# flynn-nrg/izpi

Hardware: AMD Instinct MI355X
Metric: Msamples/sec (pixels x spp) at 1024x1024/512spp (higher is better)
Workload: dtype f64

## Files before the change

### include/izpi_gpu_debug.h

```cpp
#ifndef IZPI_GPU_DEBUG_H
#define IZPI_GPU_DEBUG_H
#include "izpi_gpu.h"

#ifdef __cplusplus
extern "C" {
#endif

int izpi_gpu_debug_fault(izpi_ctx* ctx, int where);

int izpi_gpu_debug_realloc(izpi_ctx* ctx, uint32_t mask);

#ifdef __cplusplus
}
#endif
#endif
```

### izpi_amd/_native.py

```python
import ctypes as C
from pathlib import Path

ROOT = Path(__file__).resolve().parents[1]
LIB_PATH = ROOT / "izpi_amd" / "_lib" / "libizpi_gpu.so"

c_double_p = C.POINTER(C.c_double)
c_uint32_p = C.POINTER(C.c_uint32)
c_float_p = C.POINTER(C.c_float)

COMM_ID_BYTES = 128
IZPI_OK, IZPI_ERR_INVALID, IZPI_ERR_HIP, IZPI_ERR_NO_SCENE, IZPI_ERR_UNSUPPORTED, IZPI_ERR_DEVICE, IZPI_ERR_PEER = range(7)
IZPI_ABI_VERSION = 4
ACC_RECURSIVE, ACC_FORWARD = 0, 1
SCENE_QUANTIZED_BVH = 1
PRIM_TRIANGLE, PRIM_SPHERE = 0, 1
TEX_CONSTANT, TEX_IMAGE, TEX_SPECTRAL_GAUSSIAN, TEX_SPECTRAL_TABULATED, TEX_SPECTRAL_IMAGE = 1, 3, 5, 7, 9
MAT_DIELECTRIC, MAT_DIFFUSE_LIGHT, MAT_ISOTROPIC, MAT_LAMBERT, MAT_METAL, MAT_PBR = 1, 2, 3, 4, 5, 6
MATF_BEER_LAMBERT = 1
SAMPLER_NORMAL, SAMPLER_COLOUR, SAMPLER_WIREFRAME, SAMPLER_ALBEDO, SAMPLER_SPECTRAL = 1, 2, 3, 4, 5
OUT_CANVAS, OUT_PACKED = 0, 1
POST_NONE, POST_SPECTRAL, POST_GAMMA_CLAMP = 0, 1, 2
SNAP_CANVAS, SNAP_DISPLAY, SNAP_NOISE = 0, 1, 2
PROG_NOISE = 1
PROG_ADAPTIVE = 4
# ... 206 lines not shown
    _fields_ = [("name", C.c_char_p), ("kd", C.c_double * 3), ("ka", C.c_double * 3), ("ks", C.c_double * 3),
                ("num_kd", C.c_uint32), ("num_ka", C.c_uint32), ("num_ks", C.c_uint32), ("pad", C.c_uint32),
                ("ns", C.c_double), ("ni", C.c_double), ("d", C.c_double), ("sharpness", C.c_int64),
                ("illum", C.c_int64)]


ABI_STRUCTS = [BVH4Node, Texture, Material, Camera, SceneDesc, RenderReq, RenderStats, Hit, TriIn, SphereIn, CameraIn,
               SceneInput, ProtoInfo, ObjInfo, ObjGroup, ObjMaterial, RenderTuning, DenoiseParams, NoiseParams, NoiseStats, AdaptStats]

EXPORTS = [
    "izpi_gpu_open", "izpi_gpu_close", "izpi_gpu_prepare", "izpi_gpu_multi_prepare", "izpi_gpu_last_error", "izpi_gpu_upload_scene", "izpi_gpu_render",
    "izpi_gpu_render_device", "izpi_gpu_unpack_tiles", "izpi_gpu_output_bytes", "izpi_gpu_trace",
    "izpi_gpu_ray_aabb4", "izpi_gpu_gomath", "izpi_gpu_spectral_post", "izpi_gpu_postprocess",
    "izpi_gpu_build_bvh4", "izpi_gpu_multi_open", "izpi_gpu_multi_close", "izpi_gpu_multi_last_error",
    "izpi_gpu_multi_size", "izpi_gpu_multi_context", "izpi_gpu_multi_upload_scene", "izpi_gpu_multi_render",
    "izpi_gpu_comm_id", "izpi_gpu_comm_init", "izpi_gpu_render_rank", "izpi_gpu_debug_fault", "izpi_gpu_debug_realloc", "izpi_gpu_progress", "izpi_gpu_multi_progress", "izpi_host_build_scene_ex", "izpi_host_scene_prim_boxes", "izpi_host_scene_set_bvh", "izpi_host_scene_set_flags",
    "izpi_host_build_scene", "izpi_host_scene_desc", "izpi_host_scene_stack_bound", "izpi_host_scene_build_ms",
    "izpi_host_scene_free", "izpi_host_last_error", "izpi_host_tiles", "izpi_host_share_units", "izpi_host_share_tiles", "izpi_host_share_block", "izpi_host_assemble_shares", "izpi_host_bvh_leaf_max", "izpi_host_gomath", "izpi_abi_struct_size",
    "izpi_scene_parse_text", "izpi_scene_parse_binary", "izpi_scene_serialize", "izpi_scene_info", "izpi_scene_image_file",
    "izpi_scene_set_image", "izpi_scene_add_triangles", "izpi_scene_background", "izpi_scene_to_input",
    "izpi_scene_material_name", "izpi_scene_free", "izpi_light_source", "izpi_light_source_name",
    "izpi_obj_parse", "izpi_obj_info_get", "izpi_obj_copy_vertices", "izpi_obj_group_get", "izpi_obj_copy_faces",
    "izpi_obj_material_get", "izpi_obj_translate", "izpi_obj_scale", "izpi_obj_rotate",
    "izpi_obj_group_to_triangles", "izpi_obj_free",
    "izpi_gpu_displace", "izpi_host_displace", "izpi_scene_displacement_file", "izpi_scene_set_displacement_map",
    "izpi_scene_set_displacer",
    "izpi_gpu_progressive_begin", "izpi_gpu_progressive_step", "izpi_gpu_progressive_snapshot",
    "izpi_gpu_progressive_snapshot_device", "izpi_gpu_progressive_end",
    "izpi_gpu_multi_progressive_begin", "izpi_gpu_multi_progressive_step", "izpi_gpu_multi_progressive_snapshot",
    "izpi_gpu_multi_progressive_end",
    "izpi_gpu_denoise_device", "izpi_gpu_denoise", "izpi_host_denoise",
# ... 40 lines not shown
    L.izpi_gpu_multi_open.argtypes = [C.POINTER(C.c_int), C.c_uint32, C.POINTER(C.c_void_p)]
    L.izpi_gpu_multi_close.argtypes = [C.c_void_p]
    L.izpi_gpu_multi_last_error.argtypes = [C.c_void_p]
    L.izpi_gpu_multi_last_error.restype = C.c_char_p
    L.izpi_gpu_multi_size.argtypes = [C.c_void_p]
    L.izpi_gpu_multi_size.restype = C.c_uint32
    L.izpi_gpu_multi_context.argtypes = [C.c_void_p, C.c_uint32]
    L.izpi_gpu_multi_context.restype = C.c_void_p
    L.izpi_gpu_multi_upload_scene.argtypes = [C.c_void_p, C.POINTER(SceneDesc)]
    L.izpi_gpu_multi_render.argtypes = [C.c_void_p, C.POINTER(RenderReq), C.c_void_p, C.POINTER(RenderStats)]
    L.izpi_gpu_comm_id.argtypes = [C.POINTER(C.c_uint8)]
    L.izpi_gpu_comm_init.argtypes = [C.c_void_p, C.c_uint32, C.c_uint32, C.POINTER(C.c_uint8)]
    L.izpi_gpu_render_rank.argtypes = [C.c_void_p, C.POINTER(RenderReq), C.c_void_p, C.POINTER(RenderStats)]
    L.izpi_gpu_debug_fault.argtypes = [C.c_void_p, C.c_int]
    L.izpi_gpu_debug_realloc.argtypes = [C.c_void_p, C.c_uint32]
    L.izpi_gpu_progress.argtypes = [C.c_void_p, C.POINTER(C.c_uint64), C.POINTER(C.c_uint64)]
    L.izpi_gpu_multi_progress.argtypes = [C.c_void_p, C.POINTER(C.c_uint64), C.POINTER(C.c_uint64)]
    for pre in ("izpi_gpu_progressive_", "izpi_gpu_multi_progressive_"):
        getattr(L, pre + "begin").argtypes = [C.c_void_p, C.POINTER(RenderReq), C.c_uint32]
        getattr(L, pre + "step").argtypes = [C.c_void_p, C.c_uint32, C.POINTER(RenderStats)]
        getattr(L, pre + "snapshot").argtypes = [C.c_void_p, C.c_uint32, C.c_void_p]
        getattr(L, pre + "end").argtypes = [C.c_void_p]
        getattr(L, pre + "begin_ex").argtypes = [C.c_void_p, C.POINTER(RenderReq), C.c_uint32, C.c_uint32]
        getattr(L, pre + "noise").argtypes = [C.c_void_p, C.POINTER(NoiseParams), C.POINTER(NoiseStats)]
        getattr(L, pre + "adapt").argtypes = [C.c_void_p, C.POINTER(NoiseParams), C.POINTER(AdaptStats)]
        getattr(L, pre + "converge").argtypes = [C.c_void_p, C.POINTER(NoiseParams), C.POINTER(RenderStats),
                                                 C.POINTER(NoiseStats)]
    L.izpi_gpu_progressive_snapshot_device.argtypes = [C.c_void_p, C.c_uint32, C.c_void_p]
    L.izpi_host_build_scene_ex.argtypes = [C.POINTER(SceneInput), C.c_uint32, C.POINTER(C.c_void_p)]
    L.izpi_host_scene_prim_boxes.argtypes = [C.c_void_p, c_double_p]
# ... 79 lines not shown
```

### izpi_amd/csrc/components.hip

```cpp
#include "izpi_runtime.h"

using namespace izpi_internal;

__global__ void __launch_bounds__(256) k_spectral_post(const double* in, double* out, uint32_t W, uint32_t H,
                                                       double exposure) {
  __shared__ double ys[18][18];
  const int tx = threadIdx.x & 15, ty = threadIdx.x >> 4;
  const int x0 = blockIdx.x * 16, y0 = blockIdx.y * 16;
  for (int i = threadIdx.x; i < 18 * 18; i += 256) {
    const int hx = x0 + (i % 18) - 1, hy = y0 + (i / 18) - 1;
    ys[i / 18][i % 18] = (hx >= 0 && hx < (int)W && hy >= 0 && hy < (int)H) ? in[((size_t)hy * W + hx) * 4 + 1] : 0.0;
  }
  __syncthreads();
  const int x = x0 + tx, y = y0 + ty;
  if (x >= (int)W || y >= (int)H) return;
  const size_t pi = ((size_t)y * W + x) * 4;
  const double2 xy = *reinterpret_cast<const double2*>(in + pi), za = *reinterpret_cast<const double2*>(in + pi + 2);
  double X = xy.x, Y = xy.y, Z = za.x;
  const double cur = ys[ty + 1][tx + 1];
  if (cur > 0) {
    double nb[8];
    int nn = 0;
    for (int dy = -1; dy <= 1; dy++)
      for (int dx = -1; dx <= 1; dx++) {
// ... 85 lines not shown
  }
  out[i] = h;
}

__global__ void k_aabb4(const float* boxes, const float* rays, uint32_t n, uint8_t* masks) {
  const uint32_t i = blockIdx.x * 256 + threadIdx.x;
  if (i >= n) return;
  const float* b = boxes + (size_t)i * 24;
  const float* r = rays + (size_t)i * 7;
  uint8_t m = 0;
  for (int k = 0; k < 4; k++)
    if (slab(b[k], b[4 + k], b[8 + k], b[12 + k], b[16 + k], b[20 + k], r[0], r[1], r[2], r[3], r[4], r[5], r[6])) m |= (uint8_t)(1 << k);
  masks[i] = m;
}

__global__ void k_gomath(const DevScene sc, int op, const double* x, const double* y, uint32_t n, double* out) {
  const uint32_t i = blockIdx.x * 256 + threadIdx.x;
  if (i >= n) return;
  if (op == 14) {
    out[i] = path_length(mk(x[3 * i], x[3 * i + 1], x[3 * i + 2]), mk(y[3 * i], y[3 * i + 1], y[3 * i + 2]));
    return;
  }
  double a = x[i], b = y ? y[i] : 0.0, r;
  switch (op) {
    case 0: r = gm::sin(a); break;
    case 1: r = gm::cos(a); break;
    case 2: r = gm::tan(a); break;
    case 3: r = gm::exp(a); break;
    case 4: r = gm::log(a); break;
    case 5: r = gm::pow(a, b); break;
// ... 165 lines not shown
  HIP_TRY(hipSetDevice(ctx->device));
  DevBufs tmp;
  float *db, *dr; uint8_t* dm;
  HIP_TRY(tmp.alloc(&db, (size_t)n * 24));
  HIP_TRY(tmp.alloc(&dr, (size_t)n * 7));
  HIP_TRY(tmp.alloc(&dm, n));
  HIP_TRY(hipMemcpy(db, boxes, (size_t)n * 24 * sizeof(float), hipMemcpyHostToDevice));
  HIP_TRY(hipMemcpy(dr, rays, (size_t)n * 7 * sizeof(float), hipMemcpyHostToDevice));
  hipLaunchKernelGGL(k_aabb4, dim3((n + 255) / 256), dim3(256), 0, ctx->stream, db, dr, n, dm);
  HIP_TRY(hipGetLastError());
  HIP_TRY(hipStreamSynchronize(ctx->stream));
  HIP_TRY(hipMemcpy(masks, dm, n, hipMemcpyDeviceToHost));
  return IZPI_OK;
}

int izpi_gpu_gomath(izpi_ctx* ctx, int op, const double* x, const double* y, uint32_t n, double* out) {
  if (!ctx || !x || !out) return IZPI_ERR_INVALID;
  if (n == 0) return IZPI_OK;
  if (op == 37) {
    if (!ctx->have_scene) { ctx->err = "texture lookup before izpi_gpu_upload_scene"; return IZPI_ERR_NO_SCENE; }
    if (!y) { ctx->err = "texture lookup without texture numbers"; return IZPI_ERR_INVALID; }
    for (uint32_t i = 0; i < n; i++)
      if (!(y[i] >= 0 && y[i] < (double)ctx->num_textures)) { ctx->err = "texture number out of range"; return IZPI_ERR_INVALID; }
  }
  if (op == 14 && !y) { ctx->err = "path length without exit points"; return IZPI_ERR_INVALID; }
  const size_t nin = op == 14 ? 3 * (size_t)n : n;
  HIP_TRY(hipSetDevice(ctx->device));
  DevBufs tmp;
  double *dx, *dy = nullptr, *dout;
  HIP_TRY(tmp.alloc(&dx, nin));
// ... 15 lines not shown
```

### izpi_amd/csrc/izpi_dev.h

```cpp
#pragma once
#include <hip/hip_runtime.h>
#include <stdint.h>
#include "../../include/izpi_gpu.h"
#include "gomath.h"
#include "scene_records.h"

#define IZPI_DEV __device__ __forceinline__

namespace izd {

struct DevScene {
  const GInner* inner;
  const GInnerQ* innerq;
  const GLeaf* leaves;
  const GPrim* prims;
  const GShade* shade;
  const GTriTex* tritex;
  const GLight* lights;
  const izpi_material* materials;
  const izpi_texture* textures;
  const double4* mat_const;
  const MatTex* mat_tex;
  const double* texels;
  const double* spd_wl;
  const double* spd_val;
  int32_t root;
  uint32_t num_lights;
  uint32_t nan_free_bounds;
  uint32_t leaf_shortcut;
  uint32_t tri_only;
  uint32_t no_pathlen;
  uint32_t num_inner;
  uint32_t num_prims;
  izpi_camera cam;
  uint32_t lds_bytes;
  uint32_t time_free;
  uint32_t quantized;
  uint32_t addr32;
  uint32_t leaf_max;
#ifdef IZPI_SHADOW
  const GInner* sh_inner;
  const GLeaf* sh_leaves;
  const GPrim* sh_prims;
#endif
};

struct RenderParams {
  uint32_t width, height, spp, max_depth;
  uint32_t chunk_spp;
  uint32_t s0;
  uint32_t num_pixels;
  uint32_t tile_w, tile_h;
  uint32_t total_units;
  uint32_t lanes;
// ... 99 lines not shown
  double phi = 6.283185307179586 * r1;
  double sp, cp;
  gm::sincos_nonneg(phi, &sp, &cp);
  double x = cp * gm::sqrt(1 - z * z);
  double y = sp * gm::sqrt(1 - z * z);
  return mk(x, y, z);
}
IZPI_DEV V3 random_in_unit_sphere(Lcg& r) {
  for (;;) {
    double x = r.next(), y = r.next(), z = r.next();
    V3 p = sub(smul(mk(x, y, z), 2.0), mk(1.0, 1.0, 1.0));
    if (sqlen(p) < 1.0) return p;
  }
}

IZPI_DEV float max32(float a, float b) { return a > b ? a : b; }
IZPI_DEV float min32(float a, float b) { return a < b ? a : b; }
IZPI_DEV bool slab(float mnx, float mny, float mnz, float mxx, float mxy, float mxz, float ox, float oy, float oz,
                   float ix, float iy, float iz, float tmax) {
  float t0x = (mnx - ox) * ix, t1x = (mxx - ox) * ix;
  if (t0x > t1x) { float t = t0x; t0x = t1x; t1x = t; }
  float t0y = (mny - oy) * iy, t1y = (mxy - oy) * iy;
  if (t0y > t1y) { float t = t0y; t0y = t1y; t1y = t; }
  float t0z = (mnz - oz) * iz, t1z = (mxz - oz) * iz;
  if (t0z > t1z) { float t = t0z; t0z = t1z; t1z = t; }
  float tn = max32(max32(t0x, t0y), t0z);
  float tf = min32(min32(t1x, t1y), t1z);
  return tn <= tf && tf >= 0 && tn <= tmax;
}

typedef float f32x2 __attribute__((ext_vector_type(2)));
IZPI_DEV void slab4_fast(float4 mnx, float4 mny, float4 mnz, float4 mxx, float4 mxy, float4 mxz, float ox, float oy,
                         float oz, float ix, float iy, float iz, float tmax, uint64_t (&h)[4]) {
  const f32x2 o_x = {ox, ox}, o_y = {oy, oy}, o_z = {oz, oz};
  const f32x2 i_x = {ix, ix}, i_y = {iy, iy}, i_z = {iz, iz};
  const f32x2 a0x = (f32x2{mnx.x, mnx.y} - o_x) * i_x, a1x = (f32x2{mnx.z, mnx.w} - o_x) * i_x;
  const f32x2 b0x = (f32x2{mxx.x, mxx.y} - o_x) * i_x, b1x = (f32x2{mxx.z, mxx.w} - o_x) * i_x;
  const f32x2 a0y = (f32x2{mny.x, mny.y} - o_y) * i_y, a1y = (f32x2{mny.z, mny.w} - o_y) * i_y;
  const f32x2 b0y = (f32x2{mxy.x, mxy.y} - o_y) * i_y, b1y = (f32x2{mxy.z, mxy.w} - o_y) * i_y;
  const f32x2 a0z = (f32x2{mnz.x, mnz.y} - o_z) * i_z, a1z = (f32x2{mnz.z, mnz.w} - o_z) * i_z;
  const f32x2 b0z = (f32x2{mxz.x, mxz.y} - o_z) * i_z, b1z = (f32x2{mxz.z, mxz.w} - o_z) * i_z;
  const float t0x[4] = {a0x.x, a0x.y, a1x.x, a1x.y}, t1x[4] = {b0x.x, b0x.y, b1x.x, b1x.y};
  const float t0y[4] = {a0y.x, a0y.y, a1y.x, a1y.y}, t1y[4] = {b0y.x, b0y.y, b1y.x, b1y.y};
  const float t0z[4] = {a0z.x, a0z.y, a1z.x, a1z.y}, t1z[4] = {b0z.x, b0z.y, b1z.x, b1z.y};
#pragma unroll
  for (int i = 0; i < 4; i++) {
    const float tn = __builtin_fmaxf(__builtin_fmaxf(__builtin_fminf(t0x[i], t1x[i]), __builtin_fminf(t0y[i], t1y[i])),
                                     __builtin_fminf(t0z[i], t1z[i]));
    const float tf = __builtin_fminf(__builtin_fminf(__builtin_fmaxf(t0x[i], t1x[i]), __builtin_fmaxf(t0y[i], t1y[i])),
                                     __builtin_fmaxf(t0z[i], t1z[i]));
    h[i] = __builtin_amdgcn_ballot_w64(tn <= tf) & __builtin_amdgcn_ballot_w64(tf >= 0.0f) & __builtin_amdgcn_ballot_w64(tn <= tmax);
  }
}
IZPI_DEV bool ray_fast_ok(float ox, float oy, float oz, float ix, float iy, float iz) {
  const float inf = __builtin_huge_valf();
  return __builtin_fabsf(ox) < inf && __builtin_fabsf(oy) < inf && __builtin_fabsf(oz) < inf &&
         __builtin_fabsf(ix) < inf && __builtin_fabsf(iy) < inf && __builtin_fabsf(iz) < inf &&
         ix != 0.0f && iy != 0.0f && iz != 0.0f;
}

IZPI_DEV bool tri_intersect(const double* a, V3 o, V3 d, double tmin, double tmax, double& t, double& u, double& v) {
  const double eps = 1e-8;
  V3 v0 = mk(a[0], a[1], a[2]), e1 = mk(a[3], a[4], a[5]), e2 = mk(a[6], a[7], a[8]);
  V3 h = cross(d, e2);
  double aa = dot(e1, h);
  if (gm::abs(aa) < eps) return false;
  double f = 1.0 / aa;
  V3 s = sub(o, v0);
  u = f * dot(s, h);
  if (u < -eps || u > 1.0 + eps) return false;
  V3 q = cross(s, e1);
  v = f * dot(d, q);
  if (v < -eps || u + v > 1.0 + eps) return false;
// ... 53 lines not shown
```

### izpi_amd/csrc/izpi_gpu.hip

```cpp
#include "izpi_runtime.h"
#include "scene_pack.h"

#include <array>

using namespace izpi_internal;

__global__ void __launch_bounds__(256) k_cpart_reduce(const unsigned long long* cpart, uint32_t rows,
                                                      unsigned long long* counters) {
  __shared__ unsigned long long red[256];
  unsigned long long v = 0;
  for (uint32_t r = threadIdx.x; r < rows; r += 256) v += cpart[(size_t)r * CNT_N + blockIdx.x];
  red[threadIdx.x] = v;
  __syncthreads();
  for (uint32_t h = 128; h > 0; h >>= 1) {
    if (threadIdx.x < h) red[threadIdx.x] += red[threadIdx.x + h];
    __syncthreads();
  }
  if (threadIdx.x == 0) counters[blockIdx.x] += red[0];
}

namespace izpi_internal {
int grow(izpi_ctx* ctx, void** p, size_t* cap, size_t bytes) {
  if (*cap >= bytes) return IZPI_OK;
  if (*p) HIP_TRY(hipFree(*p));
// ... 488 lines not shown
  HIP_TRY(hipSetDevice(ctx->device));
  HIP_TRY(hipStreamSynchronize(ctx->stream));
  free_scene(ctx);
  return IZPI_OK;
}

int upload_packed(izpi_ctx* ctx, const izpi_scene_desc* d, const PackedScene& ps) {
  DevScene& sc = ctx->sc;
  memset(&sc, 0, sizeof(sc));
  GInner* di; GInnerQ* dq; GLeaf* dl; GPrim* dp; GShade* dsh; GTriVerts* dtv; GTriTex* dtt; GLight* dlt;
  izpi_material* dm; Double4* dmc; MatTex* dmt; izpi_texture* dtx;
  double *dtex, *dswl, *dsv;
  {
    const TraceLayout tl = trace_layout(ps.inner.size(), ps.innerq.size(), ps.leaves.size());
    char* nb;
    UP((const char*)nullptr, tl.bytes, &nb);
    di = reinterpret_cast<GInner*>(nb);
    dq = ps.innerq.empty() ? nullptr : reinterpret_cast<GInnerQ*>(nb + tl.innerq_at);
    dl = reinterpret_cast<GLeaf*>(nb + tl.leaves_at);
    HIP_TRY(hipMemcpy(di, ps.inner.data(), ps.inner.size() * sizeof(GInner), hipMemcpyHostToDevice));
    if (dq) HIP_TRY(hipMemcpy(dq, ps.innerq.data(), ps.innerq.size() * sizeof(GInnerQ), hipMemcpyHostToDevice));
    HIP_TRY(hipMemcpy(dl, ps.leaves.data(), ps.leaves.size() * sizeof(GLeaf), hipMemcpyHostToDevice));
  }
  UP(ps.prims.data(), ps.prims.size(), &dp);
  UP(ps.shade.data(), ps.shade.size(), &dsh);
  UP(ps.triverts.data(), ps.triverts.size(), &dtv);
  UP(ps.tritex.data(), ps.tritex.size(), &dtt);
  UP(ps.lights.data(), ps.lights.size(), &dlt);
  UP(d->materials, d->num_materials, &dm);
  UP(ps.mat_const.data(), ps.mat_const.size(), &dmc);
  UP(ps.mat_tex.data(), ps.mat_tex.size(), &dmt);
// ... 3 lines not shown
  UP(d->spd_values, d->num_spd, &dsv);
#ifdef IZPI_SHADOW
  {
    GInner* si; GLeaf* sl; GPrim* sp;
    UP(ps.inner.data(), ps.inner.size(), &si);
    UP(ps.leaves.data(), ps.leaves.size(), &sl);
    UP(ps.prims.data(), ps.prims.size(), &sp);
    sc.sh_inner = si; sc.sh_leaves = sl; sc.sh_prims = sp;
  }
#endif
  sc.inner = di; sc.innerq = dq; sc.leaves = dl; sc.prims = dp; sc.shade = dsh; sc.tritex = dtt; sc.lights = dlt;
  sc.materials = dm; sc.mat_const = (const double4*)dmc; sc.mat_tex = dmt; sc.textures = dtx; sc.texels = dtex;
  sc.spd_wl = dswl; sc.spd_val = dsv;
  sc.root = ps.root; sc.num_inner = ps.num_inner; sc.num_prims = d->num_prims; sc.num_lights = d->num_lights;
  sc.quantized = ps.quantized; sc.leaf_shortcut = ps.leaf_shortcut; sc.nan_free_bounds = ps.nan_free_bounds;
  sc.tri_only = ps.tri_only; sc.time_free = ps.time_free; sc.no_pathlen = ps.no_pathlen; sc.leaf_max = ps.leaf_max;
  sc.addr32 = trace_addr32(ps.inner.size(), ps.innerq.size(), ps.leaves.size(), ps.prims.size());
  sc.cam = d->camera;
  ctx->d_triverts = dtv;
  ctx->mat_ok_rgb = ps.mat_ok_rgb; ctx->mat_ok_spectral = ps.mat_ok_spectral;
  ctx->basic_materials = ps.basic_materials; ctx->matset = ps.matset;
  ctx->const_albedo = ps.const_albedo; ctx->any_uv = ps.any_uv;
  ctx->pool_grow = 0;
  ctx->stack_needed = ps.stack_needed;
  ctx->num_prims = d->num_prims;
  ctx->num_textures = d->num_textures;
  ctx->num_materials = d->num_materials;
  ctx->num_spd = d->num_spd;
  ctx->have_scene = true;
  ctx->plans[0].valid = ctx->plans[1].valid = false;
// ... 150 lines not shown
```

### izpi_amd/csrc/scene_pack.cpp

```cpp
#include "scene_pack.h"

#include <string.h>
#include <algorithm>
#include <cmath>

namespace izpi_internal {

using namespace izd;

bool stack_bound(const izpi_bvh4_node* nodes, size_t n, uint32_t* bound) {
  std::vector<uint32_t> best(n, 0);
  for (size_t k = n; k-- > 0;) {
    const izpi_bvh4_node& nd = nodes[k];
    if (nd.prim_count[0] > 0) continue;
    uint32_t valid = 0, deepest = 0;
    for (int i = 0; i < 4; i++) {
      if (nd.child[i] < 0) continue;
      valid++;
      if ((uint32_t)nd.child[i] <= k) return false;
      deepest = std::max(deepest, best[(size_t)nd.child[i]]);
    }
    best[k] = (valid ? valid - 1 : 0) + deepest;
  }
  *bound = n ? best[0] : 0;
// ... 351 lines not shown
    const double* c0 = d->sph_center0 + 3 * (size_t)i;
    const double* c1 = d->sph_center1 + 3 * (size_t)i;
    const double t0 = d->sph_time[2 * (size_t)i], t1 = d->sph_time[2 * (size_t)i + 1];
    for (int k = 0; k < 3; k++)
      if (!std::isfinite(c0[k]) || memcmp(c0 + k, c1 + k, sizeof(double)) != 0) tf = false;
    if (!std::isfinite(t0) || !std::isfinite(t1) || !(t1 > t0) || !(tmin_cam >= t0)) tf = false;
  }
  out->time_free = tf ? 1u : 0u;
  out->nan_free_bounds = 1;
  for (const GInner& g : out->inner) {
    const float* f = g.mnx;
    for (int i = 0; i < 24; i++) if (f[i] != f[i]) out->nan_free_bounds = 0;
  }
  for (const GLeaf& L : out->leaves)
    for (int i = 0; i < 3; i++) if (L.mn[i] != L.mn[i] || L.mx[i] != L.mx[i]) out->nan_free_bounds = 0;
}

}

int pack_scene(const izpi_scene_desc* d, PackedScene* out, std::string* err) {
  *out = PackedScene();
  std::vector<int32_t> ref;
  std::vector<uint32_t> mflags;
  int rc = split_bvh(d, out, ref, err);
  if (!rc) quantize_bvh(d, out);
  if (!rc) rc = pack_prims(d, out, err);
  if (!rc) rc = pack_lights(d, out, err);
  if (!rc) rc = classify_materials(d, out, mflags, err);
  if (!rc) rc = finish_shade(d, out, mflags, err);
  if (!rc) rc = pack_textures(d, out, err);
// ... 8 lines not shown
```

### izpi_amd/csrc/scene_pack.h

```cpp
#pragma once
#include <stddef.h>
#include <stdint.h>
#include <string>
#include <vector>

#include "scene_records.h"

namespace izpi_internal {

struct Double4 { double x, y, z, w; };

struct PackedScene {
  std::vector<izd::GInner> inner;
  std::vector<izd::GInnerQ> innerq;
  std::vector<izd::GLeaf> leaves;
  std::vector<izd::GPrim> prims;
  std::vector<izd::GShade> shade;
  std::vector<izd::GTriVerts> triverts;
  std::vector<izd::GTriTex> tritex;
  std::vector<izd::GLight> lights;
  std::vector<Double4> mat_const;
  std::vector<izd::MatTex> mat_tex;
  std::vector<izpi_texture> textures;
  std::vector<double> texels;
  int32_t root = -1;
  uint32_t num_inner = 0, leaf_shortcut = 1, quantized = 0, nan_free_bounds = 1, time_free = 1, no_pathlen = 1, tri_only = 1;
  uint32_t stack_needed = 0;
  uint32_t leaf_max = 0;
  bool mat_ok_rgb = true, mat_ok_spectral = true;
  bool basic_materials = true;
  uint32_t matset = 0;
  bool const_albedo = true;
  bool any_uv = false;
};

int pack_scene(const izpi_scene_desc* d, PackedScene* out, std::string* err);

struct TraceLayout { uint64_t innerq_at, leaves_at, bytes; };
inline TraceLayout trace_layout(uint64_t n_inner, uint64_t n_innerq, uint64_t n_leaves) {
  TraceLayout t;
  t.innerq_at = n_inner * sizeof(izd::GInner);
  t.leaves_at = t.innerq_at + n_innerq * sizeof(izd::GInnerQ);
  t.bytes = t.leaves_at + n_leaves * sizeof(izd::GLeaf);
  return t;
}
inline bool trace_addr32(uint64_t n_inner, uint64_t n_innerq, uint64_t n_leaves, uint64_t n_prims) {
  const uint64_t lim = 1ull << 32;
  return trace_layout(n_inner, n_innerq, n_leaves).bytes <= lim && n_prims * sizeof(izd::GPrim) <= lim;
}

bool stack_bound(const izpi_bvh4_node* nodes, size_t n, uint32_t* bound);

}
```

### izpi_amd/csrc/trace.hip

```cpp
#include "izpi_runtime.h"

constexpr uint32_t BVH_LDS_BYTES = 4096;
__device__ __forceinline__ bool lane_of(uint64_t mask) { return __builtin_amdgcn_inverse_ballot_w64(mask); }
__device__ __forceinline__ uint32_t lanes_below(uint64_t mask) {
  return __builtin_amdgcn_mbcnt_hi((uint32_t)(mask >> 32), __builtin_amdgcn_mbcnt_lo((uint32_t)mask, 0u));
}
template <int S, int WPE, bool DIST, bool TRI, bool LB, bool RL, bool Q, bool A32, bool L3, bool FT>
__global__ void __launch_bounds__(256) __attribute__((amdgpu_waves_per_eu(WPE))) k_trace2(const DevScene sc, const WaveParams wp, unsigned long long* counters,
                                                uint32_t* err, int32_t* spill, uint32_t spill_stride, uint32_t prim_w,
                                                uint32_t tchunk, uint32_t refill_min) {
  static_assert((S & (S - 1)) == 0, "ring size must be a power of two");
  static_assert(!LB || DIST, "the LDS-resident BVH instance runs the distributed leaf tests");
  static_assert(!RL || (DIST && (TRI || LB)), "the LDS-resident ray instances: triangle-only global BVH, or the BVH in LDS");
  static_assert(!Q || !LB, "the quantised nodes are read from global memory");
  static_assert(!A32 || !LB, "the 32-bit offsets address records in global memory");
  static_assert(!L3 || DIST, "the leaf size bound shapes the distributed primitive step");
  static_assert(!FT || L3, "the fixed tMin is compiled for the three-primitive leaf instances");
  constexpr uint32_t LEAF_MAX = L3 ? 3 : 4;
  constexpr bool UVL = !RL, UVS = RL && LB, DUV = !RL || LB;
  typedef float v4f __attribute__((ext_vector_type(4)));
  typedef double v2d __attribute__((ext_vector_type(2)));
  typedef const __attribute__((address_space(3))) v4f LF4;
  typedef const __attribute__((address_space(3))) v2d LD2;
  __shared__ float4 bvh_lds[LB ? BVH_LDS_BYTES / 16 : 1];
  LF4* const l_inner = (LF4*)bvh_lds;
  LF4* const l_leaves = l_inner + (size_t)8 * (LB ? sc.num_inner : 0);
  LD2* const l_prims = (LD2*)(l_leaves + (size_t)2 * (LB ? sc.num_prims : 0));
  if constexpr (LB) {
    const uint32_t ni = 8 * sc.num_inner, nl = 2 * sc.num_prims, np5 = 5 * sc.num_prims;
    for (uint32_t t = threadIdx.x; t < ni + nl + np5; t += 256)
      bvh_lds[t] = t < ni ? reinterpret_cast<const float4*>(sc.inner)[t]
                          : (t < ni + nl ? reinterpret_cast<const float4*>(sc.leaves)[t - ni]
                                         : reinterpret_cast<const float4*>(sc.prims)[t - ni - nl]);
// ... 23 lines not shown
  if ((uint64_t)(blockIdx.x * 4u + (threadIdx.x >> 6)) * first >= n) return;
  uint64_t c_rays = 0, c_nodes = 0, c_tri = 0, c_sph = 0;
  uint64_t c_nstep = 0, c_pstep = 0, c_short = 0;
  uint64_t m_scan = 0;
  bool exhausted = false;
  uint32_t qi = 0;
  uint32_t lkind = RAY_MAIN;
  double tmax = 0;
  float ix = 0, iy = 0, iz = 0, ox = 0, oy = 0, oz = 0;
  int32_t cur = -1, pk = 0, pend = 0;
  int32_t lref = 0;
  int sp = -1, low = 0;
  int clean_from = 0;
  int32_t bprim = -1;
  bool fast = false;
  uint64_t m_slow = ~0ull;
  bool any_spill = false;
#ifdef IZPI_SHADOW
  uint64_t c_spill_st = 0, c_spill_ld = 0;
  uint32_t sh_acc = 0;
#endif
  uint32_t c_pos = __builtin_amdgcn_readfirstlane((blockIdx.x * 4u + (threadIdx.x >> 6)) * first);
  uint32_t c_end = c_pos + first < n ? c_pos + first : n;
#ifdef IZPI_TRACE_CLOCKS
  uint64_t k_refill = 0, k_node = 0, k_prim = 0, k_adv = 0, k0 = 0, k1 = 0;
#define IZPI_CLK(v) (v) = __builtin_readcyclecounter()
#else
#define IZPI_CLK(v) (void)0
#endif
#ifdef IZPI_STEP_MARKS
// ... 44 lines not shown
            r = sld(wp.in.ray + my);
            const double2* rp = reinterpret_cast<const double2*>(&r);
            const double2 r0 = rp[0], r1 = rp[1], r2 = rp[2];
            ray_lds[3 * threadIdx.x] = r0; ray_lds[3 * threadIdx.x + 1] = r1; ray_lds[3 * threadIdx.x + 2] = r2;
          } else {
            r = wp.in.ray[my];
          }
          if (!(k & (RAY_PARKED | RAY_DEAD)) && (uint64_t)__double_as_longlong(r.o[0]) != DEAD_BITS) {
            qi = my;
            lkind = k;
            tmax = ray_tmax(wp.in, my, k);
            main_ray = kind_of(k) == RAY_MAIN;
            ix = (float)(1.0 / r.d[0]); iy = (float)(1.0 / r.d[1]); iz = (float)(1.0 / r.d[2]);
            ox = (float)r.o[0]; oy = (float)r.o[1]; oz = (float)r.o[2];
            fast = sc.nan_free_bounds && ray_fast_ok(ox, oy, oz, ix, iy, iz);
            cur = sc.root;
            sp = cur != -1 ? 0 : -1; low = 0; clean_from = 0;
            bprim = -1;
            if (cur == -1) {
              if ((UVL || UVS) && wp.hit_uv) {
                double2* rec = wp.in.hit + ((size_t)my << 1);
                sst(rec, hit_pack(0.0, -1)); sst(rec + 1, make_double2(0.0, 0.0));
              } else {
                sst(wp.in.hit + my, hit_pack(0.0, -1));
              }
            }
          }
        }
        c_rays += (uint64_t)__popcll(__ballot(main_ray));
        m_slow = __ballot(!fast);
// ... 191 lines not shown
            gsp[(size_t)low * spill_stride] = stk[(low & (S - 1)) * 256];
            low++;
#ifdef IZPI_SHADOW
            c_spill_st++;
#endif
          }
        }
      }
      IZPI_MARK("node_loads");
      const uint64_t m_inner = __builtin_amdgcn_ballot_w64(cur >= -1);
      if (lane_of(m_node)) {
        const float tm = (float)tmax;
        const bool is_leaf = ref_is_leaf(cur);
        float4 q0, q1, mnz_, mxx_, mxy_, mxz_;
        int4 ch_;
        const float4 *lp = nullptr, *np = nullptr;
        if constexpr (!LB && A32) {
          const uint32_t noff = is_leaf ? 0u : (uint32_t)cur * NODE_BYTES;
          const uint32_t loff = is_leaf ? leaf_off0 + (uint32_t)leaf_start(cur) * (uint32_t)sizeof(GLeaf) : noff;
          lp = reinterpret_cast<const float4*>(nbase + loff);
          np = reinterpret_cast<const float4*>(nbase + noff);
        } else if constexpr (!LB) {
          lp = reinterpret_cast<const float4*>(is_leaf ? (const void*)(sc.leaves + leaf_start(cur))
                                                       : Q ? (const void*)(sc.innerq + cur) : (const void*)(sc.inner + cur));
          np = is_leaf ? reinterpret_cast<const float4*>(nbase) : lp;
        }
        if constexpr (LB) {
          LF4* llp = is_leaf ? l_leaves + (size_t)2 * leaf_start(cur) : l_inner + (size_t)8 * cur;
          LF4* lnp = is_leaf ? l_inner : llp;
          const v4f a0 = llp[0], a1 = llp[1], a2 = lnp[2], a3 = lnp[3], a4 = lnp[4], a5 = lnp[5], c = lnp[6];
          q0 = make_float4(a0.x, a0.y, a0.z, a0.w); q1 = make_float4(a1.x, a1.y, a1.z, a1.w);
          mnz_ = make_float4(a2.x, a2.y, a2.z, a2.w); mxx_ = make_float4(a3.x, a3.y, a3.z, a3.w);
          mxy_ = make_float4(a4.x, a4.y, a4.z, a4.w); mxz_ = make_float4(a5.x, a5.y, a5.z, a5.w);
          ch_ = make_int4(__float_as_int(c.x), __float_as_int(c.y), __float_as_int(c.z), __float_as_int(c.w));
// ... 4 lines not shown
          const float sx = __uint_as_float((ex & 0xFFu) << 23), sy = __uint_as_float(((ex >> 8) & 0xFFu) << 23),
                      sz = __uint_as_float(((ex >> 16) & 0xFFu) << 23);
          auto dec4 = [](float w, float o, float sc_) {
            const uint32_t b = __float_as_uint(w);
            return make_float4(__builtin_fmaf((float)(b & 0xFFu), sc_, o), __builtin_fmaf((float)((b >> 8) & 0xFFu), sc_, o),
                               __builtin_fmaf((float)((b >> 16) & 0xFFu), sc_, o), __builtin_fmaf((float)(b >> 24), sc_, o));
          };
          const float4 dmnx = dec4(q1.x, q0.x, sx), dmny = dec4(q1.y, q0.y, sy), dmnz = dec4(q1.z, q0.z, sz);
          const float4 dmxx = dec4(q1.w, q0.x, sx), dmxy = dec4(c2.x, q0.y, sy), dmxz = dec4(c2.y, q0.z, sz);
          const float4 l0 = q0, l1 = q1;
          q0 = is_leaf ? l0 : dmnx;
          q1 = is_leaf ? l1 : make_float4(dmny.x, dmny.y, dmny.z, dmny.w);
          mnz_ = dmnz; mxx_ = dmxx; mxy_ = dmxy; mxz_ = dmxz;
          ch_ = make_int4(__float_as_int(c2.z), __float_as_int(c2.w), __float_as_int(c3.x), __float_as_int(c3.y));
        } else {
          q0 = lp[0]; q1 = lp[1];
          mnz_ = np[2]; mxx_ = np[3]; mxy_ = np[4]; mxz_ = np[5];
          ch_ = *reinterpret_cast<const int4*>(np + 6);
#ifdef IZPI_SHADOW
          if ((IZPI_SHADOW & 1) && !is_leaf) {
            const uint4* sq = reinterpret_cast<const uint4*>(sc.sh_inner + cur);
            const uint4 s0 = sq[0], s1 = sq[1], s2 = sq[2], s3 = sq[3], s4 = sq[4], s5 = sq[5], s6 = sq[6];
            sh_acc ^= s0.x ^ s1.y ^ s2.z ^ s3.w ^ s4.x ^ s5.y ^ s6.z;
          }
          if ((IZPI_SHADOW & 2) && is_leaf) {
            const uint4* sq = reinterpret_cast<const uint4*>(sc.sh_leaves + leaf_start(cur));
            const uint4 s0 = sq[0], s1 = sq[1];
            sh_acc ^= s0.x ^ s1.y;
          }
#endif
        }
        const float4 mnx = q0;
        const float4 mny = make_float4(is_leaf ? q0.y : q1.x, q1.y, q1.z, q1.w);
        const float4 mnz = make_float4(is_leaf ? q0.z : mnz_.x, mnz_.y, mnz_.z, mnz_.w);
        const float4 mxx = make_float4(is_leaf ? q0.w : mxx_.x, mxx_.y, mxx_.z, mxx_.w);
        const float4 mxy = make_float4(is_leaf ? q1.x : mxy_.x, mxy_.y, mxy_.z, mxy_.w);
        const float4 mxz = make_float4(is_leaf ? q1.y : mxz_.x, mxz_.y, mxz_.z, mxz_.w);
        const int4 ch = make_int4(is_leaf ? cur : ch_.x, ch_.y, ch_.z, ch_.w);
        uint64_t hit[4];
        if (wave_fast) {
          IZPI_MARK("slab_fast");
          slab4_fast(mnx, mny, mnz, mxx, mxy, mxz, ox, oy, oz, ix, iy, iz, tm, hit);
        } else {
          IZPI_MARK("slab_twin");
          const float amnx[4] = {mnx.x, mnx.y, mnx.z, mnx.w}, amny[4] = {mny.x, mny.y, mny.z, mny.w},
                      amnz[4] = {mnz.x, mnz.y, mnz.z, mnz.w}, amxx[4] = {mxx.x, mxx.y, mxx.z, mxx.w},
                      amxy[4] = {mxy.x, mxy.y, mxy.z, mxy.w}, amxz[4] = {mxz.x, mxz.y, mxz.z, mxz.w};
#pragma unroll
          for (int i = 0; i < 4; i++)
            hit[i] = __builtin_amdgcn_ballot_w64(slab(amnx[i], amny[i], amnz[i], amxx[i], amxy[i], amxz[i], ox, oy, oz, ix, iy, iz, tm));
        }
        IZPI_MARK("node_tail");
        const uint64_t b0 = hit[0] & __builtin_amdgcn_ballot_w64(ch.x != -1),
                       b1 = hit[1] & m_inner & __builtin_amdgcn_ballot_w64(ch.y != -1),
                       b2 = hit[2] & m_inner & __builtin_amdgcn_ballot_w64(ch.z != -1),
                       b3 = hit[3] & m_inner & __builtin_amdgcn_ballot_w64(ch.w != -1);
        next = lane_of(b3) ? ch.w : -1;
// ... 199 lines not shown
```

Measured before the change: 2677.

## Pre-sort slab planes by ray direction sign to skip per-node min/max swaps

Result: faster. 2741, median of 6 (+2.4%).

```diff
diff --git a/include/izpi_gpu_debug.h b/include/izpi_gpu_debug.h
--- a/include/izpi_gpu_debug.h
+++ b/include/izpi_gpu_debug.h
@@ -10,6 +10,8 @@
 
 int izpi_gpu_debug_realloc(izpi_ctx* ctx, uint32_t mask);
 
+int izpi_gpu_debug_slab4(izpi_ctx* ctx, const float* boxes, const float* rays, uint32_t n, uint8_t* masks);
+
 #ifdef __cplusplus
 }
 #endif
diff --git a/izpi_amd/_native.py b/izpi_amd/_native.py
--- a/izpi_amd/_native.py
+++ b/izpi_amd/_native.py
@@ -244,7 +244,7 @@
     "izpi_gpu_ray_aabb4", "izpi_gpu_gomath", "izpi_gpu_spectral_post", "izpi_gpu_postprocess",
     "izpi_gpu_build_bvh4", "izpi_gpu_multi_open", "izpi_gpu_multi_close", "izpi_gpu_multi_last_error",
     "izpi_gpu_multi_size", "izpi_gpu_multi_context", "izpi_gpu_multi_upload_scene", "izpi_gpu_multi_render",
-    "izpi_gpu_comm_id", "izpi_gpu_comm_init", "izpi_gpu_render_rank", "izpi_gpu_debug_fault", "izpi_gpu_debug_realloc", "izpi_gpu_progress", "izpi_gpu_multi_progress", "izpi_host_build_scene_ex", "izpi_host_scene_prim_boxes", "izpi_host_scene_set_bvh", "izpi_host_scene_set_flags",
+    "izpi_gpu_comm_id", "izpi_gpu_comm_init", "izpi_gpu_render_rank", "izpi_gpu_debug_fault", "izpi_gpu_debug_realloc", "izpi_gpu_debug_slab4", "izpi_gpu_progress", "izpi_gpu_multi_progress", "izpi_host_build_scene_ex", "izpi_host_scene_prim_boxes", "izpi_host_scene_set_bvh", "izpi_host_scene_set_flags",
     "izpi_host_build_scene", "izpi_host_scene_desc", "izpi_host_scene_stack_bound", "izpi_host_scene_build_ms",
     "izpi_host_scene_free", "izpi_host_last_error", "izpi_host_tiles", "izpi_host_share_units", "izpi_host_share_tiles", "izpi_host_share_block", "izpi_host_assemble_shares", "izpi_host_bvh_leaf_max", "izpi_host_gomath", "izpi_abi_struct_size",
     "izpi_scene_parse_text", "izpi_scene_parse_binary", "izpi_scene_serialize", "izpi_scene_info", "izpi_scene_image_file",
@@ -315,6 +315,7 @@
     L.izpi_gpu_render_rank.argtypes = [C.c_void_p, C.POINTER(RenderReq), C.c_void_p, C.POINTER(RenderStats)]
     L.izpi_gpu_debug_fault.argtypes = [C.c_void_p, C.c_int]
     L.izpi_gpu_debug_realloc.argtypes = [C.c_void_p, C.c_uint32]
+    L.izpi_gpu_debug_slab4.argtypes = [C.c_void_p, c_float_p, c_float_p, C.c_uint32, C.POINTER(C.c_uint8)]
     L.izpi_gpu_progress.argtypes = [C.c_void_p, C.POINTER(C.c_uint64), C.POINTER(C.c_uint64)]
     L.izpi_gpu_multi_progress.argtypes = [C.c_void_p, C.POINTER(C.c_uint64), C.POINTER(C.c_uint64)]
     for pre in ("izpi_gpu_progressive_", "izpi_gpu_multi_progressive_"):
diff --git a/izpi_amd/csrc/components.hip b/izpi_amd/csrc/components.hip
--- a/izpi_amd/csrc/components.hip
+++ b/izpi_amd/csrc/components.hip
@@ -123,6 +123,36 @@
   masks[i] = m;
 }
 
+__global__ void k_debug_slab4(const float* boxes, const float* rays, uint32_t n, uint8_t* masks) {
+  const uint32_t i = blockIdx.x * 256 + threadIdx.x;
+  const uint32_t j = i < n ? i : n - 1;
+  const float* b = boxes + (size_t)j * 24;
+  const float* r = rays + (size_t)j * 7;
+  const float ox = r[0], oy = r[1], oz = r[2], ix = r[3], iy = r[4], iz = r[5], tm = r[6];
+  bool box_ok = true;
+  for (int k = 0; k < 4; k++) box_ok = box_ok && b[k] <= b[12 + k] && b[4 + k] <= b[16 + k] && b[8 + k] <= b[20 + k];
+  const bool fast = box_ok && ray_fast_ok(ox, oy, oz, ix, iy, iz);
+  const uint32_t nx = slab_near_index(0, ix, fast), ny = slab_near_index(1, iy, fast), nz = slab_near_index(2, iz, fast);
+  auto plane = [&](uint32_t k) { return make_float4(b[4 * k], b[4 * k + 1], b[4 * k + 2], b[4 * k + 3]); };
+  const float4 p0 = plane(nx), p1 = plane(ny), p2 = plane(nz);
+  const float4 p3 = plane(slab_far_index(0, nx)), p4 = plane(slab_far_index(1, ny)), p5 = plane(slab_far_index(2, nz));
+  uint64_t hit[4];
+  if (__builtin_amdgcn_ballot_w64(!fast) == 0) {
+    slab4_sorted(p0, p1, p2, p3, p4, p5, ox, oy, oz, ix, iy, iz, tm, hit);
+  } else {
+    const float a0[4] = {p0.x, p0.y, p0.z, p0.w}, a1[4] = {p1.x, p1.y, p1.z, p1.w}, a2[4] = {p2.x, p2.y, p2.z, p2.w},
+                a3[4] = {p3.x, p3.y, p3.z, p3.w}, a4[4] = {p4.x, p4.y, p4.z, p4.w}, a5[4] = {p5.x, p5.y, p5.z, p5.w};
+#pragma unroll
+    for (int k = 0; k < 4; k++)
+      hit[k] = __builtin_amdgcn_ballot_w64(slab(a0[k], a1[k], a2[k], a3[k], a4[k], a5[k], ox, oy, oz, ix, iy, iz, tm));
+  }
+  const uint32_t lane = threadIdx.x & 63;
+  uint8_t m = 0;
+#pragma unroll
+  for (int k = 0; k < 4; k++) m |= (uint8_t)(((hit[k] >> lane) & 1u) << k);
+  if (i < n) masks[i] = m;
+}
+
 __global__ void k_gomath(const DevScene sc, int op, const double* x, const double* y, uint32_t n, double* out) {
   const uint32_t i = blockIdx.x * 256 + threadIdx.x;
   if (i >= n) return;
@@ -318,6 +348,24 @@
   return IZPI_OK;
 }
 
+int izpi_gpu_debug_slab4(izpi_ctx* ctx, const float* boxes, const float* rays, uint32_t n, uint8_t* masks) {
+  if (!ctx || !boxes || !rays || !masks) return IZPI_ERR_INVALID;
+  if (n == 0) return IZPI_OK;
+  HIP_TRY(hipSetDevice(ctx->device));
+  DevBufs tmp;
+  float *db, *dr; uint8_t* dm;
+  HIP_TRY(tmp.alloc(&db, (size_t)n * 24));
+  HIP_TRY(tmp.alloc(&dr, (size_t)n * 7));
+  HIP_TRY(tmp.alloc(&dm, n));
+  HIP_TRY(hipMemcpy(db, boxes, (size_t)n * 24 * sizeof(float), hipMemcpyHostToDevice));
+  HIP_TRY(hipMemcpy(dr, rays, (size_t)n * 7 * sizeof(float), hipMemcpyHostToDevice));
+  hipLaunchKernelGGL(k_debug_slab4, dim3((n + 255) / 256), dim3(256), 0, ctx->stream, db, dr, n, dm);
+  HIP_TRY(hipGetLastError());
+  HIP_TRY(hipStreamSynchronize(ctx->stream));
+  HIP_TRY(hipMemcpy(masks, dm, n, hipMemcpyDeviceToHost));
+  return IZPI_OK;
+}
+
 int izpi_gpu_gomath(izpi_ctx* ctx, int op, const double* x, const double* y, uint32_t n, double* out) {
   if (!ctx || !x || !out) return IZPI_ERR_INVALID;
   if (n == 0) return IZPI_OK;
diff --git a/izpi_amd/csrc/izpi_dev.h b/izpi_amd/csrc/izpi_dev.h
--- a/izpi_amd/csrc/izpi_dev.h
+++ b/izpi_amd/csrc/izpi_dev.h
@@ -4,6 +4,7 @@
 #include "../../include/izpi_gpu.h"
 #include "gomath.h"
 #include "scene_records.h"
+#include "slab_rule.h"
 
 #define IZPI_DEV __device__ __forceinline__
 
@@ -38,6 +39,7 @@
   uint32_t quantized;
   uint32_t addr32;
   uint32_t leaf_max;
+  uint32_t ordered_bounds;
 #ifdef IZPI_SHADOW
   const GInner* sh_inner;
   const GLeaf* sh_leaves;
@@ -167,20 +169,6 @@
   }
 }
 
-IZPI_DEV float max32(float a, float b) { return a > b ? a : b; }
-IZPI_DEV float min32(float a, float b) { return a < b ? a : b; }
-IZPI_DEV bool slab(float mnx, float mny, float mnz, float mxx, float mxy, float mxz, float ox, float oy, float oz,
-                   float ix, float iy, float iz, float tmax) {
-  float t0x = (mnx - ox) * ix, t1x = (mxx - ox) * ix;
-  if (t0x > t1x) { float t = t0x; t0x = t1x; t1x = t; }
-  float t0y = (mny - oy) * iy, t1y = (mxy - oy) * iy;
-  if (t0y > t1y) { float t = t0y; t0y = t1y; t1y = t; }
-  float t0z = (mnz - oz) * iz, t1z = (mxz - oz) * iz;
-  if (t0z > t1z) { float t = t0z; t0z = t1z; t1z = t; }
-  float tn = max32(max32(t0x, t0y), t0z);
-  float tf = min32(min32(t1x, t1y), t1z);
-  return tn <= tf && tf >= 0 && tn <= tmax;
-}
 
 typedef float f32x2 __attribute__((ext_vector_type(2)));
 IZPI_DEV void slab4_fast(float4 mnx, float4 mny, float4 mnz, float4 mxx, float4 mxy, float4 mxz, float ox, float oy,
@@ -205,11 +193,24 @@
     h[i] = __builtin_amdgcn_ballot_w64(tn <= tf) & __builtin_amdgcn_ballot_w64(tf >= 0.0f) & __builtin_amdgcn_ballot_w64(tn <= tmax);
   }
 }
-IZPI_DEV bool ray_fast_ok(float ox, float oy, float oz, float ix, float iy, float iz) {
-  const float inf = __builtin_huge_valf();
-  return __builtin_fabsf(ox) < inf && __builtin_fabsf(oy) < inf && __builtin_fabsf(oz) < inf &&
-         __builtin_fabsf(ix) < inf && __builtin_fabsf(iy) < inf && __builtin_fabsf(iz) < inf &&
-         ix != 0.0f && iy != 0.0f && iz != 0.0f;
+IZPI_DEV void slab4_sorted(float4 nrx, float4 nry, float4 nrz, float4 frx, float4 fry, float4 frz, float ox, float oy,
+                           float oz, float ix, float iy, float iz, float tmax, uint64_t (&h)[4]) {
+  const f32x2 o_x = {ox, ox}, o_y = {oy, oy}, o_z = {oz, oz};
+  const f32x2 i_x = {ix, ix}, i_y = {iy, iy}, i_z = {iz, iz};
+  const f32x2 a0x = (f32x2{nrx.x, nrx.y} - o_x) * i_x, a1x = (f32x2{nrx.z, nrx.w} - o_x) * i_x;
+  const f32x2 b0x = (f32x2{frx.x, frx.y} - o_x) * i_x, b1x = (f32x2{frx.z, frx.w} - o_x) * i_x;
+  const f32x2 a0y = (f32x2{nry.x, nry.y} - o_y) * i_y, a1y = (f32x2{nry.z, nry.w} - o_y) * i_y;
+  const f32x2 b0y = (f32x2{fry.x, fry.y} - o_y) * i_y, b1y = (f32x2{fry.z, fry.w} - o_y) * i_y;
+  const f32x2 a0z = (f32x2{nrz.x, nrz.y} - o_z) * i_z, a1z = (f32x2{nrz.z, nrz.w} - o_z) * i_z;
+  const f32x2 b0z = (f32x2{frz.x, frz.y} - o_z) * i_z, b1z = (f32x2{frz.z, frz.w} - o_z) * i_z;
+  const float nx[4] = {a0x.x, a0x.y, a1x.x, a1x.y}, fx[4] = {b0x.x, b0x.y, b1x.x, b1x.y};
+  const float ny[4] = {a0y.x, a0y.y, a1y.x, a1y.y}, fy[4] = {b0y.x, b0y.y, b1y.x, b1y.y};
+  const float nz[4] = {a0z.x, a0z.y, a1z.x, a1z.y}, fz[4] = {b0z.x, b0z.y, b1z.x, b1z.y};
+#pragma unroll
+  for (int i = 0; i < 4; i++) {
+    const float tn = slab_sorted_near(nx[i], ny[i], nz[i]), tf = slab_sorted_far(fx[i], fy[i], fz[i]);
+    h[i] = __builtin_amdgcn_ballot_w64(tn <= tf) & __builtin_amdgcn_ballot_w64(tf >= 0.0f) & __builtin_amdgcn_ballot_w64(tn <= tmax);
+  }
 }
 
 IZPI_DEV bool tri_intersect(const double* a, V3 o, V3 d, double tmin, double tmax, double& t, double& u, double& v) {
diff --git a/izpi_amd/csrc/izpi_gpu.hip b/izpi_amd/csrc/izpi_gpu.hip
--- a/izpi_amd/csrc/izpi_gpu.hip
+++ b/izpi_amd/csrc/izpi_gpu.hip
@@ -526,7 +526,7 @@
   {
     const TraceLayout tl = trace_layout(ps.inner.size(), ps.innerq.size(), ps.leaves.size());
     char* nb;
-    UP((const char*)nullptr, tl.bytes, &nb);
+    UP((const char*)nullptr, tl.alloc_bytes, &nb);
     di = reinterpret_cast<GInner*>(nb);
     dq = ps.innerq.empty() ? nullptr : reinterpret_cast<GInnerQ*>(nb + tl.innerq_at);
     dl = reinterpret_cast<GLeaf*>(nb + tl.leaves_at);
@@ -560,6 +560,7 @@
   sc.spd_wl = dswl; sc.spd_val = dsv;
   sc.root = ps.root; sc.num_inner = ps.num_inner; sc.num_prims = d->num_prims; sc.num_lights = d->num_lights;
   sc.quantized = ps.quantized; sc.leaf_shortcut = ps.leaf_shortcut; sc.nan_free_bounds = ps.nan_free_bounds;
+  sc.ordered_bounds = ps.ordered_bounds;
   sc.tri_only = ps.tri_only; sc.time_free = ps.time_free; sc.no_pathlen = ps.no_pathlen; sc.leaf_max = ps.leaf_max;
   sc.addr32 = trace_addr32(ps.inner.size(), ps.innerq.size(), ps.leaves.size(), ps.prims.size());
   sc.cam = d->camera;
diff --git a/izpi_amd/csrc/scene_pack.cpp b/izpi_amd/csrc/scene_pack.cpp
--- a/izpi_amd/csrc/scene_pack.cpp
+++ b/izpi_amd/csrc/scene_pack.cpp
@@ -389,6 +389,12 @@
   }
   for (const GLeaf& L : out->leaves)
     for (int i = 0; i < 3; i++) if (L.mn[i] != L.mn[i] || L.mx[i] != L.mx[i]) out->nan_free_bounds = 0;
+  out->ordered_bounds = 1;
+  for (const GInner& g : out->inner)
+    for (int i = 0; i < 4; i++)
+      if (g.child[i] != -1 && !(g.mnx[i] <= g.mxx[i] && g.mny[i] <= g.mxy[i] && g.mnz[i] <= g.mxz[i])) out->ordered_bounds = 0;
+  for (const GLeaf& L : out->leaves)
+    for (int i = 0; i < 3; i++) if (!(L.mn[i] <= L.mx[i])) out->ordered_bounds = 0;
 }
 
 }
diff --git a/izpi_amd/csrc/scene_pack.h b/izpi_amd/csrc/scene_pack.h
--- a/izpi_amd/csrc/scene_pack.h
+++ b/izpi_amd/csrc/scene_pack.h
@@ -24,7 +24,7 @@
   std::vector<izpi_texture> textures;
   std::vector<double> texels;
   int32_t root = -1;
-  uint32_t num_inner = 0, leaf_shortcut = 1, quantized = 0, nan_free_bounds = 1, time_free = 1, no_pathlen = 1, tri_only = 1;
+  uint32_t num_inner = 0, leaf_shortcut = 1, quantized = 0, nan_free_bounds = 1, ordered_bounds = 1, time_free = 1, no_pathlen = 1, tri_only = 1;
   uint32_t stack_needed = 0;
   uint32_t leaf_max = 0;
   bool mat_ok_rgb = true, mat_ok_spectral = true;
@@ -36,12 +36,14 @@
 
 int pack_scene(const izpi_scene_desc* d, PackedScene* out, std::string* err);
 
-struct TraceLayout { uint64_t innerq_at, leaves_at, bytes; };
+constexpr uint64_t TRACE_TAIL_PAD = 16;
+struct TraceLayout { uint64_t innerq_at, leaves_at, bytes, alloc_bytes; };
 inline TraceLayout trace_layout(uint64_t n_inner, uint64_t n_innerq, uint64_t n_leaves) {
   TraceLayout t;
   t.innerq_at = n_inner * sizeof(izd::GInner);
   t.leaves_at = t.innerq_at + n_innerq * sizeof(izd::GInnerQ);
   t.bytes = t.leaves_at + n_leaves * sizeof(izd::GLeaf);
+  t.alloc_bytes = t.bytes + TRACE_TAIL_PAD;
   return t;
 }
 inline bool trace_addr32(uint64_t n_inner, uint64_t n_innerq, uint64_t n_leaves, uint64_t n_prims) {
diff --git a/izpi_amd/csrc/slab_rule.h b/izpi_amd/csrc/slab_rule.h
--- /dev/null
+++ b/izpi_amd/csrc/slab_rule.h
@@ -0,0 +1,49 @@
+#pragma once
+#include <stdint.h>
+
+#if defined(__HIP__)
+#define IZPI_SR __host__ __device__ __forceinline__
+#else
+#define IZPI_SR inline
+#endif
+
+namespace izd {
+
+IZPI_SR float max32(float a, float b) { return a > b ? a : b; }
+IZPI_SR float min32(float a, float b) { return a < b ? a : b; }
+IZPI_SR bool slab(float mnx, float mny, float mnz, float mxx, float mxy, float mxz, float ox, float oy, float oz,
+                  float ix, float iy, float iz, float tmax) {
+  float t0x = (mnx - ox) * ix, t1x = (mxx - ox) * ix;
+  if (t0x > t1x) { float t = t0x; t0x = t1x; t1x = t; }
+  float t0y = (mny - oy) * iy, t1y = (mxy - oy) * iy;
+  if (t0y > t1y) { float t = t0y; t0y = t1y; t1y = t; }
+  float t0z = (mnz - oz) * iz, t1z = (mxz - oz) * iz;
+  if (t0z > t1z) { float t = t0z; t0z = t1z; t1z = t; }
+  float tn = max32(max32(t0x, t0y), t0z);
+  float tf = min32(min32(t1x, t1y), t1z);
+  return tn <= tf && tf >= 0 && tn <= tmax;
+}
+
+IZPI_SR bool ray_fast_ok(float ox, float oy, float oz, float ix, float iy, float iz) {
+  const float inf = __builtin_huge_valf();
+  return __builtin_fabsf(ox) < inf && __builtin_fabsf(oy) < inf && __builtin_fabsf(oz) < inf &&
+         __builtin_fabsf(ix) < inf && __builtin_fabsf(iy) < inf && __builtin_fabsf(iz) < inf &&
+         ix != 0.0f && iy != 0.0f && iz != 0.0f;
+}
+
+IZPI_SR uint32_t slab_near_index(uint32_t axis, float inv, bool fast) { return axis + ((fast && inv < 0.0f) ? 3u : 0u); }
+IZPI_SR uint32_t slab_far_index(uint32_t axis, uint32_t near) { return 3u + 2u * axis - near; }
+
+IZPI_SR float slab_sorted_near(float nx, float ny, float nz) { return __builtin_fmaxf(__builtin_fmaxf(nx, ny), nz); }
+IZPI_SR float slab_sorted_far(float fx, float fy, float fz) { return __builtin_fminf(__builtin_fminf(fx, fy), fz); }
+IZPI_SR bool slab_sorted_hit(float nx, float ny, float nz, float fx, float fy, float fz, float tmax) {
+  const float tn = slab_sorted_near(nx, ny, nz), tf = slab_sorted_far(fx, fy, fz);
+  return tn <= tf && tf >= 0 && tn <= tmax;
+}
+IZPI_SR bool slab_sorted(const float* b, uint32_t nx, uint32_t ny, uint32_t nz, float ox, float oy, float oz, float ix,
+                         float iy, float iz, float tmax) {
+  return slab_sorted_hit((b[nx] - ox) * ix, (b[ny] - oy) * iy, (b[nz] - oz) * iz, (b[slab_far_index(0, nx)] - ox) * ix,
+                         (b[slab_far_index(1, ny)] - oy) * iy, (b[slab_far_index(2, nz)] - oz) * iz, tmax);
+}
+
+}
diff --git a/izpi_amd/csrc/trace.hip b/izpi_amd/csrc/trace.hip
--- a/izpi_amd/csrc/trace.hip
+++ b/izpi_amd/csrc/trace.hip
@@ -17,6 +17,9 @@
   static_assert(!L3 || DIST, "the leaf size bound shapes the distributed primitive step");
   static_assert(!FT || L3, "the fixed tMin is compiled for the three-primitive leaf instances");
   constexpr uint32_t LEAF_MAX = L3 ? 3 : 4;
+  constexpr bool SG = !LB && !Q && (A32 || DIST || TRI);
+  constexpr bool PK = SG && !TRI;
+  typedef float v4fu __attribute__((ext_vector_type(4), aligned(4)));
   constexpr bool UVL = !RL, UVS = RL && LB, DUV = !RL || LB;
   typedef float v4f __attribute__((ext_vector_type(4)));
   typedef double v2d __attribute__((ext_vector_type(2)));
@@ -70,6 +73,7 @@
   int clean_from = 0;
   int32_t bprim = -1;
   bool fast = false;
+  uint32_t nrx = 0, nry = 1, nrz = 2, nrp = 0x020100u;
   uint64_t m_slow = ~0ull;
   bool any_spill = false;
 #ifdef IZPI_SHADOW
@@ -144,6 +148,12 @@
             ix = (float)(1.0 / r.d[0]); iy = (float)(1.0 / r.d[1]); iz = (float)(1.0 / r.d[2]);
             ox = (float)r.o[0]; oy = (float)r.o[1]; oz = (float)r.o[2];
             fast = sc.nan_free_bounds && ray_fast_ok(ox, oy, oz, ix, iy, iz);
+            if constexpr (SG) {
+              fast = fast && sc.ordered_bounds;
+              const uint32_t kx = slab_near_index(0, ix, fast), ky = slab_near_index(1, iy, fast), kz = slab_near_index(2, iz, fast);
+              if constexpr (PK) nrp = kx | (ky << 8) | (kz << 16);
+              else { nrx = kx; nry = ky; nrz = kz; }
+            }
             cur = sc.root;
             sp = cur != -1 ? 0 : -1; low = 0; clean_from = 0;
             bprim = -1;
@@ -365,10 +375,12 @@
         const bool is_leaf = ref_is_leaf(cur);
         float4 q0, q1, mnz_, mxx_, mxy_, mxz_;
         int4 ch_;
+        float4 mnx, mny, mnz, mxx, mxy, mxz;
         const float4 *lp = nullptr, *np = nullptr;
+        uint32_t loff = 0;
         if constexpr (!LB && A32) {
           const uint32_t noff = is_leaf ? 0u : (uint32_t)cur * NODE_BYTES;
-          const uint32_t loff = is_leaf ? leaf_off0 + (uint32_t)leaf_start(cur) * (uint32_t)sizeof(GLeaf) : noff;
+          loff = is_leaf ? leaf_off0 + (uint32_t)leaf_start(cur) * (uint32_t)sizeof(GLeaf) : noff;
           lp = reinterpret_cast<const float4*>(nbase + loff);
           np = reinterpret_cast<const float4*>(nbase + noff);
         } else if constexpr (!LB) {
@@ -403,8 +415,21 @@
           mnz_ = dmnz; mxx_ = dmxx; mxy_ = dmxy; mxz_ = dmxz;
           ch_ = make_int4(__float_as_int(c2.z), __float_as_int(c2.w), __float_as_int(c3.x), __float_as_int(c3.y));
         } else {
-          q0 = lp[0]; q1 = lp[1];
-          mnz_ = np[2]; mxx_ = np[3]; mxy_ = np[4]; mxz_ = np[5];
+          if constexpr (SG) {
+            const uint32_t sh = is_leaf ? 2u : 4u;
+            if constexpr (PK) { nrx = nrp & 0xFFu; nry = (nrp >> 8) & 0xFFu; nrz = nrp >> 16; }
+            const uint32_t frx = slab_far_index(0, nrx), fry = slab_far_index(1, nry), frz = slab_far_index(2, nrz);
+            auto plane = [&](uint32_t i) {
+              const v4fu v = A32 ? *reinterpret_cast<const v4fu*>(nbase + (uint32_t)((i << sh) + loff))
+                                 : *reinterpret_cast<const v4fu*>(reinterpret_cast<const char*>(lp) + (i << sh));
+              return make_float4(v.x, v.y, v.z, v.w);
+            };
+            mnx = plane(nrx); mny = plane(nry); mnz = plane(nrz);
+            mxx = plane(frx); mxy = plane(fry); mxz = plane(frz);
+          } else {
+            q0 = lp[0]; q1 = lp[1];
+            mnz_ = np[2]; mxx_ = np[3]; mxy_ = np[4]; mxz_ = np[5];
+          }
           ch_ = *reinterpret_cast<const int4*>(np + 6);
 #ifdef IZPI_SHADOW
           if ((IZPI_SHADOW & 1) && !is_leaf) {
@@ -419,17 +444,20 @@
           }
 #endif
         }
-        const float4 mnx = q0;
-        const float4 mny = make_float4(is_leaf ? q0.y : q1.x, q1.y, q1.z, q1.w);
-        const float4 mnz = make_float4(is_leaf ? q0.z : mnz_.x, mnz_.y, mnz_.z, mnz_.w);
-        const float4 mxx = make_float4(is_leaf ? q0.w : mxx_.x, mxx_.y, mxx_.z, mxx_.w);
-        const float4 mxy = make_float4(is_leaf ? q1.x : mxy_.x, mxy_.y, mxy_.z, mxy_.w);
-        const float4 mxz = make_float4(is_leaf ? q1.y : mxz_.x, mxz_.y, mxz_.z, mxz_.w);
+        if constexpr (!SG) {
+          mnx = q0;
+          mny = make_float4(is_leaf ? q0.y : q1.x, q1.y, q1.z, q1.w);
+          mnz = make_float4(is_leaf ? q0.z : mnz_.x, mnz_.y, mnz_.z, mnz_.w);
+          mxx = make_float4(is_leaf ? q0.w : mxx_.x, mxx_.y, mxx_.z, mxx_.w);
+          mxy = make_float4(is_leaf ? q1.x : mxy_.x, mxy_.y, mxy_.z, mxy_.w);
+          mxz = make_float4(is_leaf ? q1.y : mxz_.x, mxz_.y, mxz_.z, mxz_.w);
+        }
         const int4 ch = make_int4(is_leaf ? cur : ch_.x, ch_.y, ch_.z, ch_.w);
         uint64_t hit[4];
         if (wave_fast) {
           IZPI_MARK("slab_fast");
-          slab4_fast(mnx, mny, mnz, mxx, mxy, mxz, ox, oy, oz, ix, iy, iz, tm, hit);
+          if constexpr (SG) slab4_sorted(mnx, mny, mnz, mxx, mxy, mxz, ox, oy, oz, ix, iy, iz, tm, hit);
+          else slab4_fast(mnx, mny, mnz, mxx, mxy, mxz, ox, oy, oz, ix, iy, iz, tm, hit);
         } else {
           IZPI_MARK("slab_twin");
           const float amnx[4] = {mnx.x, mnx.y, mnx.z, mnx.w}, amny[4] = {mny.x, mny.y, mny.z, mny.w},
```
